# PRBonn/lidar_transfer

Measured on AMD Instinct MI355X. Metric: Mrays/sec, one new ~1M-triangle mesh per scan -> 64x2048 range/label image, higher is better.
Workload: dtype f32; 1 GPU; C2: 64x2048 rays vs 999788-triangle synthetic scene (fov 3.0/-25.0); 1 step = 64 scans, each a new mesh; 48 scenes cycled; parallelism=scan-parallel x1, scans_in_flight=24, scans_per_call=8

## Files before the change

### lidar_transfer_amd/csrc/lt_scatter.hip

```cpp
#include "lt_internal.h"
#include <math.h>
#include <stdlib.h>
#include <string.h>
#include "lt_normalize.h"

#define LT_PI_F 3.14159265358979f
#define LT_BIN_SLACK 4e-3f
#define LT_EMPTY_KEY 0xFFFFFFFFFFFFFFFFull

struct rs_params {
  int nb_az, nb_el;
  float az_scale;
  float az_off;
  float el_lo, el_scale;
  float dev_az, dev_el;
  float dev_fit[2];
  float el_c0, el_c1, az_c0, az_c1;
};

__device__ __forceinline__ float rs_az_off(float phi0, float az_scale) {
  if (!(phi0 == phi0)) return 0.f;
  const float x0 = (phi0 + LT_PI_F) * az_scale;
  return x0 - floorf(x0 + 0.5f);
}

__global__ __launch_bounds__(256) void k_rs_dirs(const float* __restrict__ rays, int n, unsigned flags,
                                                 float4* __restrict__ dirs, float2* __restrict__ ang,
                                                 float* __restrict__ partial) {
  __shared__ float red[4][2];
  float lo = INFINITY, hi = -INFINITY;
  for (int i = blockIdx.x * 256 + threadIdx.x; i < n; i += gridDim.x * 256) {
    const float rx = rays[3 * (size_t)i], ry = rays[3 * (size_t)i + 1], rz = rays[3 * (size_t)i + 2];
    const float D = (rx * rx + ry * ry) + rz * rz;
    const float r0 = lt_rsqrt_seed(D, flags);
    const float r = (1.5f * r0) + (((D * -0.5f) * r0) * (r0 * r0));
    const float dx = rx * r, dy = ry * r, dz = rz * r;
    dirs[i] = make_float4(dx, dy, dz, 0.f);
    const float phi = atan2f(dy, dx), th = atan2f(dz, sqrtf(dx * dx + dy * dy));
    ang[i] = make_float2(phi, th);
    if (th == th) { lo = fminf(lo, th); hi = fmaxf(hi, th); }
  }
#pragma unroll
  for (int o = 32; o > 0; o >>= 1) {
    lo = fminf(lo, __shfl_xor(lo, o, 64));
    hi = fmaxf(hi, __shfl_xor(hi, o, 64));
  }
  if ((threadIdx.x & 63) == 0) { red[threadIdx.x >> 6][0] = lo; red[threadIdx.x >> 6][1] = hi; }
  __syncthreads();
  if (threadIdx.x == 0) {
    partial[2 * blockIdx.x] = fminf(fminf(red[0][0], red[1][0]), fminf(red[2][0], red[3][0]));
    partial[2 * blockIdx.x + 1] = fmaxf(fmaxf(red[0][1], red[1][1]), fmaxf(red[2][1], red[3][1]));
  }
}

__global__ __launch_bounds__(256) void k_rs_fit(const float2* __restrict__ ang, int n, int nb_az0,
                                                rs_params* __restrict__ prm) {
  const float phi0 = n > 0 ? ang[0].x : 0.f;
  float dev[2] = {0.f, 0.f};
  for (int k = 0; k < 2; ++k) {
    const int K = nb_az0 - k;
    if (K < 1) continue;
    const float sc = (float)K / (2.0f * LT_PI_F), off = rs_az_off(phi0, sc);
    for (int i = blockIdx.x * 256 + threadIdx.x; i < n; i += gridDim.x * 256) {
      const float phi = ang[i].x;
      if (phi == phi) {
        const float x = (phi + LT_PI_F) * sc - off;
        dev[k] = fmaxf(dev[k], fabsf(x - floorf(x + 0.5f)));
      }
    }
  }
#pragma unroll
  for (int o = 32; o > 0; o >>= 1) {
    dev[0] = fmaxf(dev[0], __shfl_xor(dev[0], o, 64));
    dev[1] = fmaxf(dev[1], __shfl_xor(dev[1], o, 64));
  }
  if ((threadIdx.x & 63) == 0) {
    atomicMax((int*)&prm->dev_fit[0], __float_as_int(dev[0]));
    atomicMax((int*)&prm->dev_fit[1], __float_as_int(dev[1]));
  }
}

__global__ __launch_bounds__(256) void k_rs_keys(const float2* __restrict__ ang, int n, int nb_az, int nb_el,
                                                 const float* __restrict__ partial, rs_params* __restrict__ prm,
                                                 uint32_t* __restrict__ keys, uint32_t* __restrict__ vals) {
  __shared__ float red[4][2];
  float lo = partial[2 * threadIdx.x], hi = partial[2 * threadIdx.x + 1];
#pragma unroll
  for (int o = 32; o > 0; o >>= 1) {
    lo = fminf(lo, __shfl_xor(lo, o, 64));
    hi = fmaxf(hi, __shfl_xor(hi, o, 64));
  }
  if ((threadIdx.x & 63) == 0) { red[threadIdx.x >> 6][0] = lo; red[threadIdx.x >> 6][1] = hi; }
  __syncthreads();
  lo = fminf(fminf(red[0][0], red[1][0]), fminf(red[2][0], red[3][0]));
  hi = fmaxf(fmaxf(red[0][1], red[1][1]), fmaxf(red[2][1], red[3][1]));
  if (!(lo <= hi)) { lo = 0.f; hi = 0.f; }
  const int nb_max = nb_az;
  if (nb_az >= 5 && prm->dev_fit[1] + 0.01f < prm->dev_fit[0]) nb_az -= 1;
  rs_params p;
  p.nb_az = nb_az; p.nb_el = nb_el;
  p.az_scale = (float)nb_az / (2.0f * LT_PI_F);
  p.az_off = rs_az_off(n > 0 ? ang[0].x : 0.f, p.az_scale);
  p.el_lo = lo;
  p.el_scale = (nb_el > 1 && hi > lo) ? (float)(nb_el - 1) / (hi - lo) : 0.f;
  if (blockIdx.x == 0 && threadIdx.x == 0) {
    prm->nb_az = p.nb_az; prm->nb_el = p.nb_el;
    prm->az_scale = p.az_scale; prm->az_off = p.az_off; prm->el_lo = p.el_lo; prm->el_scale = p.el_scale;
  }
  const int i = blockIdx.x * 256 + threadIdx.x;
  float dev_a = 0.f, dev_e = 0.f;
  if (i < n) {
    const float2 a = ang[i];
    uint32_t key = (uint32_t)nb_max * (uint32_t)nb_el;
    if (a.x == a.x && a.y == a.y) {
      const float x = (a.x + LT_PI_F) * p.az_scale - p.az_off, y = (a.y - p.el_lo) * p.el_scale;
      const float cx = floorf(x + 0.5f);
      const float cy = fminf(fmaxf(floorf(y + 0.5f), 0.f), (float)(nb_el - 1));
      dev_a = fabsf(x - cx);
      dev_e = fabsf(y - cy);
      int ia = (int)cx;
      if (ia < 0) ia += nb_az;
      else if (ia >= nb_az) ia -= nb_az;
      ia = min(max(ia, 0), nb_az - 1);
      key = (uint32_t)cy * (uint32_t)nb_az + (uint32_t)ia;
    }
    keys[i] = key;
    vals[i] = (uint32_t)i;
  }
#pragma unroll
  for (int o = 32; o > 0; o >>= 1) {
    dev_a = fmaxf(dev_a, __shfl_xor(dev_a, o, 64));
    dev_e = fmaxf(dev_e, __shfl_xor(dev_e, o, 64));
  }
  if ((threadIdx.x & 63) == 0) {
    atomicMax((int*)&prm->dev_az, __float_as_int(dev_a));
    atomicMax((int*)&prm->dev_el, __float_as_int(dev_e));
  }
}

__global__ __launch_bounds__(256) void k_rs_starts(const uint32_t* __restrict__ keys, int n, int nbins,
                                                   int* __restrict__ bin_start) {
  const int p = blockIdx.x * 256 + threadIdx.x;
  if (p > n) return;
  const int lo = p == 0 ? 0 : (int)min(keys[p - 1], (uint32_t)nbins) + 1;
  const int hi = p == n ? nbins : (int)min(keys[p], (uint32_t)nbins);
  for (int b = lo; b <= hi; ++b) bin_start[b] = p;
}

struct tri_rec {
  float v0x, v0y, v0z, e1x, e1y, e1z, e2x, e2y, e2z;
};

__device__ __forceinline__ float sc_mt(const tri_rec& T, float ox, float oy, float oz, float dx, float dy, float dz) {
  const float eps = 0.000001f;
  const float hx = dy * T.e2z - dz * T.e2y, hy = dz * T.e2x - dx * T.e2z, hz = dx * T.e2y - dy * T.e2x;
  const float a = (T.e1x * hx + T.e1y * hy) + T.e1z * hz;
  if (a < eps && a > -eps) return NAN;
  const float inv_a = lt_rcp_ieee(a);
  const float sx = ox - T.v0x, sy = oy - T.v0y, sz = oz - T.v0z;
  const float u = ((sx * hx + sy * hy) + sz * hz) * inv_a;
  if (u < 0 || u > 1) return NAN;
  const float qx = sy * T.e1z - sz * T.e1y, qy = sz * T.e1x - sx * T.e1z, qz = sx * T.e1y - sy * T.e1x;
  const float v = ((dx * qx + dy * qy) + dz * qz) * inv_a;
  if (v < 0 || u + v > 1) return NAN;
  const float t = ((T.e2x * qx + T.e2y * qy) + T.e2z * qz) * inv_a;
  if (t < eps) return NAN;
  return t;
}

__device__ __forceinline__ float f_rcp(float x) { return __builtin_amdgcn_rcpf(x); }
__device__ __forceinline__ float f_sqrt(float x) { return __builtin_amdgcn_sqrtf(x); }
__device__ __forceinline__ float f_atan2(float y, float x) {
#pragma clang fp contract(fast)
  const float ax = fabsf(x), ay = fabsf(y);
  const float mx = fmaxf(ax, ay), mn = fminf(ax, ay);
  const float a = mx > 0.f ? mn * f_rcp(mx) : 0.f;
  const float q = a * a;
  float r = a * (0.99997726f + q * (-0.33262347f + q * (0.19354346f + q * (-0.11643287f + q * (0.05265332f + q * -0.01172120f)))));
  r = ay > ax ? 1.57079632679f - r : r;
  r = x < 0.f ? 3.14159265359f - r : r;
  return y < 0.f ? -r : r;
}

__device__ __forceinline__ void f_atan_pair(float za, float ra, float zb, float rb, float& tha, float& thb) {
#pragma clang fp contract(fast)
  const float ta = za * f_rcp(ra), tb = zb * f_rcp(rb);
  const bool easy = fabsf(ta) <= 1.0f && fabsf(tb) <= 1.0f;
  if (__ballot(!easy) == 0ull) {
    const float qa = ta * ta, qb = tb * tb;
    tha = ta * (0.99997726f + qa * (-0.33262347f + qa * (0.19354346f + qa * (-0.11643287f + qa * (0.05265332f + qa * -0.01172120f)))));
    thb = tb * (0.99997726f + qb * (-0.33262347f + qb * (0.19354346f + qb * (-0.11643287f + qb * (0.05265332f + qb * -0.01172120f)))));
  } else {
    tha = f_atan2(za, ra);
    thb = f_atan2(zb, rb);
  }
}

__device__ __forceinline__ float seg_dist2d_sq(float ax, float ay, float bx, float by) {
#pragma clang fp contract(fast)
  const float ex = bx - ax, ey = by - ay;
  const float l2 = ex * ex + ey * ey;
  float t = l2 > 0.f ? -(ax * ex + ay * ey) * f_rcp(l2) : 0.f;
  t = fminf(fmaxf(t, 0.f), 1.f);
  const float cx = ax + t * ex, cy = ay + t * ey;
  return cx * cx + cy * cy;
}

template <class T>
__device__ __forceinline__ unsigned byte_off(unsigned elem) {
  if (sizeof(T) == 12) {
    unsigned r;
    asm("v_lshl_add_u32 %0, %1, 3, %2" : "=v"(r) : "v"(elem), "v"(elem << 2));
    return r;
  }
  return elem * (unsigned)sizeof(T);
}
template <bool WIDE, class T>
__device__ __forceinline__ const T* at(const T* base, unsigned elem) {
  return WIDE ? base + (size_t)elem : (const T*)((const char*)base + byte_off<T>(elem));
}
template <bool WIDE, class T>
__device__ __forceinline__ T* at(T* base, unsigned elem) {
  return WIDE ? base + (size_t)elem : (T*)((char*)base + byte_off<T>(elem));
}
struct f3 { float x, y, z; };
struct i3 { int x, y, z; };

struct bin_rect { int a0, na, e0, e1; };

__device__ __forceinline__ bin_rect tri_bins(const rs_params& P, float x0, float y0, float z0, float x1, float y1,
                                             float z1, float x2, float y2, float z2, float e1x, float e1y, float e2x,
                                             float e2y) {
#pragma clang fp contract(fast)
  bin_rect R;
  R.na = 0;
  const float q0 = x0 * x0 + y0 * y0, q1 = x1 * x1 + y1 * y1, q2 = x2 * x2 + y2 * y2;
  if (!(q0 + q1 + q2 < 1e36f && fabsf(z0) + fabsf(z1) + fabsf(z2) < 1e18f)) {
    const float sum = ((x0 + y0) + (z0 + x1)) + ((y1 + z1) + (x2 + y2)) + z2;
    const float asum = ((fabsf(x0) + fabsf(y0)) + (fabsf(z0) + fabsf(x1))) + ((fabsf(y1) + fabsf(z1)) + (fabsf(x2) + fabsf(y2))) + fabsf(z2);
    if (sum != sum || asum == INFINITY) return R;
    R.e0 = 0; R.e1 = P.nb_el - 1; R.a0 = 0; R.na = P.nb_az;
    return R;
  }
  const float rho_max2 = fmaxf(q0, fmaxf(q1, q2));
  const float rho_max = f_sqrt(rho_max2);
  const float zmin = fminf(z0, fminf(z1, z2)), zmax = fmaxf(z0, fmaxf(z1, z2));
  const float c0 = x0 * y1 - x1 * y0, c1 = x1 * y2 - x2 * y1, c2 = x2 * y0 - x0 * y2;
  const float tol = 1e-6f * rho_max2 + 1e-12f;
  const float cmin = fminf(c0, fminf(c1, c2)), cmax = fmaxf(c0, fmaxf(c1, c2));
  const bool outside = cmin < -tol && cmax > tol;
  bool edge_on = cmin >= -tol && cmax <= tol;
  const float e12x = e2x - e1x, e12y = e2y - e1y;
  const float lmax2 = fmaxf(e1x * e1x + e1y * e1y, fmaxf(e12x * e12x + e12y * e12y, e2x * e2x + e2y * e2y));
  const float qmin = fminf(q0, fminf(q1, q2));
  float rho_edges2;
  if (__ballot(!(lmax2 <= 0.01f * qmin)) == 0ull) {
    rho_edges2 = qmin - 0.25f * lmax2;
  } else {
    rho_edges2 =
        fminf(seg_dist2d_sq(x0, y0, x1, y1), fminf(seg_dist2d_sq(x1, y1, x2, y2), seg_dist2d_sq(x2, y2, x0, y0)));
  }
  const float rho_edges = f_sqrt(rho_edges2);
  const float rho_tiny = 1e-4f * rho_max + 1e-6f;
  if (!outside && rho_edges2 > 4.0f * lmax2) edge_on = true;
  const bool pierced = !(outside || (edge_on && rho_edges > rho_tiny));
  const float rho_min = pierced ? 0.f : rho_edges;
  const float z_near = __builtin_amdgcn_fmed3f(zmin, 0.f, zmax);
  const float dlo2 = fmaxf((pierced ? 0.f : rho_edges2) + z_near * z_near, 0.0025f);
  const float pad = 3e-4f + 2e-4f * __builtin_amdgcn_rsqf(dlo2);
  const float pad_az = 3e-4f + 2e-4f * __builtin_amdgcn_rsqf(fmaxf(rho_edges2, 0.0025f));
  float th_hi, th_lo;
  f_atan_pair(zmax, zmax > 0.f ? rho_min : rho_max, zmin, zmin < 0.f ? rho_min : rho_max, th_hi, th_lo);
  th_hi += pad;
  th_lo -= pad;
  const float fe0 = ceilf(th_lo * P.el_scale + P.el_c0), fe1 = floorf(th_hi * P.el_scale + P.el_c1);
  if (!(fe1 >= 0.f) || !(fe0 <= (float)(P.nb_el - 1)) || !(fe0 <= fe1)) return R;
  R.e0 = (int)fmaxf(fe0, 0.f);
  R.e1 = (int)fminf(fe1, (float)(P.nb_el - 1));
  if (pierced || rho_min <= rho_tiny || P.nb_az < 4) {
    R.a0 = 0;
    R.na = P.nb_az;
    return R;
  }
  float a_lo, a_hi;
  if (!edge_on) {
    const bool l0 = c0 >= 0.f && c2 <= 0.f, l1 = c1 >= 0.f && c0 <= 0.f;
    const bool h0 = c0 <= 0.f && c2 >= 0.f, h1 = c1 <= 0.f && c0 >= 0.f;
    a_lo = f_atan2(l0 ? y0 : (l1 ? y1 : y2), l0 ? x0 : (l1 ? x1 : x2));
    a_hi = f_atan2(h0 ? y0 : (h1 ? y1 : y2), h0 ? x0 : (h1 ? x1 : x2));
    if (a_hi < a_lo) a_hi += 2.0f * LT_PI_F;
  } else {
    const float p0 = f_atan2(y0, x0), p1 = f_atan2(y1, x1), p2 = f_atan2(y2, x2);
    const float lo = fminf(p0, fminf(p1, p2)), hi = fmaxf(p0, fmaxf(p1, p2));
    const float mid = (p0 + p1 + p2) - lo - hi;
    const float g0 = mid - lo, g1 = hi - mid, g2 = 2.0f * LT_PI_F - (hi - lo);
    if (g2 >= g0 && g2 >= g1) { a_lo = lo; a_hi = hi; }
    else if (g0 >= g1) { a_lo = mid; a_hi = lo + 2.0f * LT_PI_F; }
    else { a_lo = hi; a_hi = mid + 2.0f * LT_PI_F; }
  }
  a_lo -= pad_az;
  a_hi += pad_az;
  const float fa0 = ceilf(a_lo * P.az_scale + P.az_c0);
  const float fa1 = floorf(a_hi * P.az_scale + P.az_c1);
  const int na = (int)(fa1 - fa0) + 1;
  if (!(na >= 1)) return R;
  if (na >= P.nb_az) { R.a0 = 0; R.na = P.nb_az; return R; }
  int a0 = (int)fa0;
  if (a0 < 0) a0 += P.nb_az;
  else if (a0 >= P.nb_az) a0 -= P.nb_az;
  R.a0 = a0;
  R.na = na;
  return R;
}

#define LT_GRID_EMPTY (-1)
#define LT_GRID_MULTI (-2)
template <bool WIDE>
__device__ __forceinline__ void sc_hit(float t, int ray, int face, unsigned long long* __restrict__ cell) {
  if (t < 999999999.f) atomicMin(at<WIDE>(cell, (unsigned)ray), ((unsigned long long)__float_as_uint(t) << 32) | (unsigned)face);
}
template <bool WIDE>
__device__ __forceinline__ void sc_test_cell(const tri_rec& T, int face, const float4 g,
                                             const float4* __restrict__ sdirs, float ox, float oy, float oz,
                                             unsigned long long* __restrict__ cell, unsigned& n_tests) {
  const int w = __float_as_int(g.w);
  if (w != LT_GRID_MULTI) {
    n_tests += w >= 0 ? 1u : 0u;
    sc_hit<WIDE>(sc_mt(T, ox, oy, oz, g.x, g.y, g.z), w, face, cell);
  } else {
    for (int k = __float_as_int(g.x), e = __float_as_int(g.y); k < e; ++k) {
      const float4 d = *at<WIDE>(sdirs, (unsigned)k);
      ++n_tests;
      sc_hit<WIDE>(sc_mt(T, ox, oy, oz, d.x, d.y, d.z), __float_as_int(d.w), face, cell);
    }
  }
}

__global__ __launch_bounds__(256) void k_rs_sortdirs(const float4* __restrict__ dirs,
                                                     const uint32_t* __restrict__ bin_rays, int n,
                                                     float4* __restrict__ sdirs) {
  const int k = blockIdx.x * 256 + threadIdx.x;
  if (k >= n) return;
  const int ray = (int)bin_rays[k];
  float4 d = dirs[ray];
  d.w = __int_as_float(ray);
  sdirs[k] = d;
}

__global__ __launch_bounds__(256) void k_rs_grid(const int* __restrict__ bin_start,
                                                 const float4* __restrict__ sdirs, int nbins,
                                                 float4* __restrict__ grid) {
  const int b = blockIdx.x * 256 + threadIdx.x;
  if (b >= nbins) return;
  const int s = bin_start[b], e = bin_start[b + 1];
  float4 g = make_float4(0.f, 0.f, 0.f, __int_as_float(LT_GRID_EMPTY));
  if (e - s == 1) g = sdirs[s];
  else if (e - s > 1) g = make_float4(__int_as_float(s), __int_as_float(e), 0.f, __int_as_float(LT_GRID_MULTI));
  grid[b] = g;
}

#define LT_SC_BIG 512
#define LT_SC_CAP_SINGLE 1536
#define LT_SC_CAP_BATCH 8192
#ifndef LT_SC_SLICE
#define LT_SC_SLICE 512
#endif

#ifndef LT_SC_T
#define LT_SC_T 448
#endif
#define LT_SC_T2 (LT_SC_T - 256)
static_assert(LT_SC_T >= 256 && LT_SC_T <= 512 && LT_SC_T2 % 64 == 0, "LT_SC_T: 256, 320, 384, 448 or 512");

struct sc_shared {
  float4 q0[LT_SC_T], q1[LT_SC_T];
  float2 q2[LT_SC_T];
  unsigned pre[513];
  unsigned wsum[4];
  int kept;
};

struct sc_one { int cnt; unsigned a0; };

template <bool PUSH>
__device__ __forceinline__ sc_one sc_record_into(float4* s_q0, float4* s_q1, float2* s_q2, int slot, int f, const f3 A,
                                                 const f3 Bv, const f3 C, float ox, float oy, float oz, const rs_params& P,
                                                 int* __restrict__ large, int* __restrict__ large_count) {
  sc_one r;
  r.cnt = 0; r.a0 = 0;
  const float v0x = A.x, v0y = A.y, v0z = A.z, v1x = Bv.x, v1y = Bv.y, v1z = Bv.z;
  const float v2x = C.x, v2y = C.y, v2z = C.z;
  const float e1x = v1x - v0x, e1y = v1y - v0y, e2x = v2x - v0x, e2y = v2y - v0y;
  const bin_rect R = tri_bins(P, v0x - ox, v0y - oy, v0z - oz, v1x - ox, v1y - oy, v1z - oz, v2x - ox, v2y - oy,
                              v2z - oz, e1x, e1y, e2x, e2y);
  if (R.na > 0) {
    const int c32 = R.na * (R.e1 - R.e0 + 1);
    if (c32 > LT_SC_BIG) {
      if (PUSH) large[atomicAdd(large_count, 1)] = f;
    } else {
      r.cnt = c32;
      r.a0 = (unsigned)R.a0;
      s_q0[slot] = make_float4(v0x, v0y, v0z, e1x);
      s_q1[slot] = make_float4(e1y, v1z - v0z, e2x, e2y);
      s_q2[slot] = make_float2(v2z - v0z, __int_as_float((R.na - 1) | (R.e0 << 9)));
    }
  }
  return r;
}
template <bool PUSH>
__device__ __forceinline__ sc_one sc_record(sc_shared& S, int slot, int f, const f3 A, const f3 Bv, const f3 C, float ox,
                                            float oy, float oz, const rs_params& P, int* __restrict__ large,
                                            int* __restrict__ large_count) {
  return sc_record_into<PUSH>(S.q0, S.q1, S.q2, slot, f, A, Bv, C, ox, oy, oz, P, large, large_count);
}

template <bool PUSH, bool WIDE>
__device__ __forceinline__ void sc_setup(sc_shared& S, const float* __restrict__ verts, const int* __restrict__ faces,
                                         int n_verts, int n_faces, int first, float ox, float oy, float oz,
                                         const rs_params& P, int* __restrict__ large, int* __restrict__ large_count,
                                         unsigned* __restrict__ flags, sc_one& rA, sc_one& rB) {
  const int tid = threadIdx.x;
  rA.cnt = 0; rA.a0 = 0; rB.cnt = 0; rB.a0 = 0;
  const int fA = first + tid, fB = first + 256 + tid;
  const bool hasA = fA < n_faces, hasB = LT_SC_T2 > 0 && tid < LT_SC_T2 && fB < n_faces;
  if (n_verts <= 0) {
    if (PUSH && (hasA || hasB)) atomicOr(flags, LT_FLAG_BAD_INDEX);
    return;
  }
  const i3 iA = *at<WIDE>((const i3*)faces, (unsigned)(hasA ? fA : 0));
  i3 iB = iA;
  if (LT_SC_T2 > 0) iB = *at<WIDE>((const i3*)faces, (unsigned)(hasB ? fB : 0));
  const unsigned nv = (unsigned)n_verts;
  const bool okA = hasA && (unsigned)iA.x < nv && (unsigned)iA.y < nv && (unsigned)iA.z < nv;
  const bool okB = hasB && (unsigned)iB.x < nv && (unsigned)iB.y < nv && (unsigned)iB.z < nv;
  const f3 A0 = *at<WIDE>((const f3*)verts, okA ? (unsigned)iA.x : 0u);
  const f3 A1 = *at<WIDE>((const f3*)verts, okA ? (unsigned)iA.y : 0u);
  const f3 A2 = *at<WIDE>((const f3*)verts, okA ? (unsigned)iA.z : 0u);
  f3 B0 = A0, B1 = A1, B2 = A2;
  if (LT_SC_T2 > 0) {
    B0 = *at<WIDE>((const f3*)verts, okB ? (unsigned)iB.x : 0u);
    B1 = *at<WIDE>((const f3*)verts, okB ? (unsigned)iB.y : 0u);
    B2 = *at<WIDE>((const f3*)verts, okB ? (unsigned)iB.z : 0u);
  }
  if (PUSH && ((hasA && !okA) || (hasB && !okB))) atomicOr(flags, LT_FLAG_BAD_INDEX);
  if (okA) rA = sc_record<PUSH>(S, tid, fA, A0, A1, A2, ox, oy, oz, P, large, large_count);
  if (LT_SC_T2 > 0 && okB) rB = sc_record<PUSH>(S, 256 + tid, fB, B0, B1, B2, ox, oy, oz, P, large, large_count);
}

__device__ __forceinline__ void sc_prefix(sc_shared& S, const sc_one rA, const sc_one rB, int& preA, int& preB, int& total) {
  const int tid = threadIdx.x, lane = tid & 63, wave = tid >> 6;
  unsigned inc = (unsigned)rA.cnt | ((unsigned)rB.cnt << 16);
  asm volatile(
      "s_nop 1\n\tv_add_u32_dpp %0, %0, %0 row_shr:1 row_mask:0xf bank_mask:0xf bound_ctrl:0\n\t"
      "s_nop 1\n\tv_add_u32_dpp %0, %0, %0 row_shr:2 row_mask:0xf bank_mask:0xf bound_ctrl:0\n\t"
      "s_nop 1\n\tv_add_u32_dpp %0, %0, %0 row_shr:4 row_mask:0xf bank_mask:0xf bound_ctrl:0\n\t"
      "s_nop 1\n\tv_add_u32_dpp %0, %0, %0 row_shr:8 row_mask:0xf bank_mask:0xf bound_ctrl:0\n\t"
      "s_nop 1\n\tv_add_u32_dpp %0, %0, %0 row_bcast:15 row_mask:0xa bank_mask:0xf\n\t"
      "s_nop 1\n\tv_add_u32_dpp %0, %0, %0 row_bcast:31 row_mask:0xc bank_mask:0xf\n\t"
      "s_nop 1"
      : "+v"(inc));
  if (lane == 63) S.wsum[wave] = inc;
  __syncthreads();
  int woffA = 0, woffB = 0, totA = 0, totB = 0;
#pragma unroll
  for (int w = 0; w < 4; ++w) {
    const unsigned ws = S.wsum[w];
    const int a = (int)(ws & 0xFFFFu), b = (int)(ws >> 16);
    if (w < wave) { woffA += a; woffB += b; }
    totA += a; totB += b;
  }
  total = totA + totB;
  preA = woffA + (int)(inc & 0xFFFFu) - rA.cnt;
  preB = totA + woffB + (int)(inc >> 16) - rB.cnt;
  S.pre[tid] = ((unsigned)preA << 13) | rA.a0;
  if (LT_SC_T2 > 0 && tid < LT_SC_T2) S.pre[256 + tid] = ((unsigned)preB << 13) | rB.a0;
  else S.pre[256 + tid] = (256 + tid == LT_SC_T) ? ((unsigned)total << 13) : 0xFFFFFFFFu;
  if (tid == 255) S.pre[512] = LT_SC_T == 512 ? ((unsigned)total << 13) : 0xFFFFFFFFu;
}

template <bool COUNT, bool WIDE, int NT, int NE>
__device__ __forceinline__ void sc_round_robin(const unsigned* s_pre, const float4* s_q0, const float4* s_q1,
                                               const float2* s_q2, const rs_params& P, const float4* __restrict__ grid,
                                               const float4* __restrict__ sdirs, unsigned long long* __restrict__ cell,
                                               int first_face, int c_begin, int c_end, int tix, float ox, float oy, float oz,
                                               unsigned& n_tests, unsigned& n_cand) {
  auto ldu = [](const unsigned* arr, unsigned j4) { return *(const unsigned*)((const char*)arr + j4); };
  auto ldq = [](const float4* arr, unsigned j4) { return *(const float4*)((const char*)arr + 4u * j4); };
  auto ld2 = [](const float2* arr, unsigned j4) { return *(const float2*)((const char*)arr + 2u * j4); };
  const unsigned pre0 = s_pre[0];
  auto locate = [&](int c, unsigned& j4, float2& q2) -> int {
    const unsigned ck = ((unsigned)c << 13) | 0x1FFFu;
    j4 = 0;
    unsigned base = pre0;
#pragma unroll
    for (unsigned step4 = 2u * NE; step4 >= 4; step4 >>= 1) {
      const unsigned v = ldu(s_pre, j4 + step4);
      const bool take = v <= ck;
      j4 = take ? j4 + step4 : j4;
      base = take ? v : base;
    }
    const int local = c - (int)(base >> 13);
    q2 = ld2(s_q2, j4);
    const int pk = __float_as_int(q2.y);
    const int na = (pk & 511) + 1;
    const int row = (int)(((float)local + 0.5f) * f_rcp((float)na));
    int az = (int)(base & 0x1FFFu) + (local - __mul24(row, na));
    if (az >= P.nb_az) az -= P.nb_az;
    return __mul24((pk >> 9) + row, P.nb_az) + az;
  };
  int c = c_begin + tix;
  if (c < c_end) {
    unsigned j4;
    float2 q2;
    float4 g = *at<false>(grid, (unsigned)locate(c, j4, q2));
    for (;;) {
      const int cn = c + NT;
      unsigned jn4 = 0;
      float2 q2n = make_float2(0.f, 0.f);
      float4 gn = make_float4(0.f, 0.f, 0.f, 0.f);
      if (__ballot(cn < c_end) != 0ull) gn = *at<false>(grid, (unsigned)locate(min(cn, c_end - 1), jn4, q2n));
      const float4 q0 = ldq(s_q0, j4), q1 = ldq(s_q1, j4);
      tri_rec T;
      T.v0x = q0.x; T.v0y = q0.y; T.v0z = q0.z;
      T.e1x = q0.w; T.e1y = q1.x; T.e1z = q1.y;
      T.e2x = q1.z; T.e2y = q1.w; T.e2z = q2.x;
      if (COUNT) ++n_cand;
      sc_test_cell<WIDE>(T, first_face + (int)(j4 >> 2), g, sdirs, ox, oy, oz, cell, n_tests);
      if (cn >= c_end) break;
      c = cn; j4 = jn4; g = gn; q2 = q2n;
    }
  }
}

template <bool COUNT>
__device__ __forceinline__ void sc_count(unsigned n_tests, unsigned n_cand, unsigned long long* __restrict__ counters) {
  if (COUNT) {
    unsigned long long vt = n_tests, vc = n_cand;
#pragma unroll
    for (int o = 32; o > 0; o >>= 1) { vt += __shfl_xor(vt, o, 64); vc += __shfl_xor(vc, o, 64); }
    if ((threadIdx.x & 63) == 0) { atomicAdd(&counters[1], vt); atomicAdd(&counters[0], vc); }
  }
}

#ifndef LT_SC_MAX_BATCH
#define LT_SC_MAX_BATCH 8
#endif
struct sc_job {
  const float* verts; const int* faces; const int* colors; const float* rem;
  rs_params P; const float4* grid; const float4* sdirs; const float4* dirs;
  unsigned long long* cell; int* large; int* large_count; int2* slices;
  unsigned* flags; unsigned long long* counters;
  float* endpoints; int* endcolors; float* range; float* endrem; int* tri;
  float ox, oy, oz;
  int n_verts, n_faces, n_rays, cap_slices;
  unsigned out_flags;
};
struct sc_batch {
  int n;
  int tris_blocks, resolve_blocks;
  int cap;
  int rest_blocks;
  int tris_block0[LT_SC_MAX_BATCH];
  int resolve_block0[LT_SC_MAX_BATCH];
  sc_job job[LT_SC_MAX_BATCH];
};
__device__ __forceinline__ int sc_find_job(const int (&block0)[LT_SC_MAX_BATCH], int block) {
  int j = 0;
#pragma unroll
  for (int k = 1; k < LT_SC_MAX_BATCH; ++k) j += block >= block0[k] ? 1 : 0;
  return j;
}


template <bool COUNT, bool WIDE>
__global__ __launch_bounds__(256) void k_sc_tris(const sc_batch B) {
  __shared__ sc_shared S;
  const int j = sc_find_job(B.tris_block0, (int)blockIdx.x);
  const sc_job& J = B.job[j];
  const int lb = (int)blockIdx.x - B.tris_block0[j];
  const int tid = threadIdx.x;
  const int first = lb * LT_SC_T;
  const rs_params P = J.P;
  const float ox = J.ox, oy = J.oy, oz = J.oz;
  sc_one rA, rB;
  sc_setup<true, WIDE>(S, J.verts, J.faces, J.n_verts, J.n_faces, first, ox, oy, oz, P, J.large, J.large_count, J.flags, rA,
                       rB);
  int total, preA, preB;
  sc_prefix(S, rA, rB, preA, preB, total);
  if (total < B.cap) {
    if (tid == 255) S.kept = total;
  } else {
    const bool crossA = preA < B.cap && preA + rA.cnt >= B.cap;
    const bool crossB = LT_SC_T2 > 0 && tid < LT_SC_T2 && preB < B.cap && preB + rB.cnt >= B.cap;
    if (crossA || crossB) {
      int kept = crossA ? preA + rA.cnt : preB + rB.cnt;
      const int n_sl = (total - kept + LT_SC_SLICE - 1) / LT_SC_SLICE;
      if (n_sl > 0) {
        const int base = atomicAdd(&J.large_count[1], n_sl);
        if (base + n_sl <= J.cap_slices) {
          for (int k = 0; k < n_sl; ++k) J.slices[base + k] = make_int2(lb, kept + k * LT_SC_SLICE);
        } else {
          atomicSub(&J.large_count[1], n_sl);
          kept = total;
        }
      }
      S.kept = kept;
    }
  }
  __syncthreads();
  const int kept = S.kept;
  unsigned n_tests = 0, n_cand = 0;
  sc_round_robin<COUNT, WIDE, 256, (LT_SC_T > 256 ? 512 : 256)>(S.pre, S.q0, S.q1, S.q2, P, J.grid, J.sdirs, J.cell, first, 0,
                                                                kept, tid, ox, oy, oz, n_tests, n_cand);
  sc_count<COUNT>(n_tests, n_cand, J.counters);
}

#define LT_SC_REST_BLOCKS 512
#define LT_SC_REST_BLOCKS_BATCH 128
#define LT_SC_PARTS 8
template <bool COUNT, bool WIDE>
__global__ __launch_bounds__(256) void k_sc_rest(const sc_batch B) {
  __shared__ sc_shared S;
  const int rest_blocks = B.rest_blocks;
  const sc_job& J = B.job[blockIdx.x / rest_blocks];
  const int rb = blockIdx.x % rest_blocks;
  if (J.n_faces <= 0) return;
  const float* __restrict__ verts = J.verts;
  const int* __restrict__ faces = J.faces;
  const float4* __restrict__ grid = J.grid;
  const float4* __restrict__ sdirs = J.sdirs;
  unsigned long long* __restrict__ cell = J.cell;
  const float ox = J.ox, oy = J.oy, oz = J.oz;
  const rs_params P = J.P;
  const int n_large = J.large_count[0], n_slices = min(J.large_count[1], J.cap_slices);
  if (COUNT && rb == 0 && threadIdx.x == 0) J.counters[3] = (unsigned long long)n_large | ((unsigned long long)n_slices << 32);
  unsigned n_tests = 0, n_cand = 0;
  for (int q = rb; q < n_slices; q += rest_blocks) {
    const int2 sl = J.slices[q];
    const int first = sl.x * LT_SC_T;
    sc_one rA, rB;
    sc_setup<false, WIDE>(S, verts, faces, J.n_verts, J.n_faces, first, ox, oy, oz, P, nullptr, nullptr, nullptr, rA, rB);
    int total, preA, preB;
    sc_prefix(S, rA, rB, preA, preB, total);
    __syncthreads();
    sc_round_robin<COUNT, WIDE, 256, (LT_SC_T > 256 ? 512 : 256)>(S.pre, S.q0, S.q1, S.q2, P, grid, sdirs, cell, first, sl.y,
                                                                  min(sl.y + LT_SC_SLICE, total), (int)threadIdx.x, ox, oy,
                                                                  oz, n_tests, n_cand);
    __syncthreads();
  }
  const int lane = threadIdx.x & 63;
  const int wave0 = rb * 4 + (threadIdx.x >> 6), nwaves = rest_blocks * 4;
  for (int v = wave0; v < n_large * LT_SC_PARTS; v += nwaves) {
    const int q = v / LT_SC_PARTS, part = v - q * LT_SC_PARTS;
    const int f = J.large[q];
    const float* pa = verts + 3 * (size_t)faces[3 * (size_t)f];
    const float* pb = verts + 3 * (size_t)faces[3 * (size_t)f + 1];
    const float* pc = verts + 3 * (size_t)faces[3 * (size_t)f + 2];
    tri_rec T;
    T.v0x = pa[0]; T.v0y = pa[1]; T.v0z = pa[2];
    const float v1x = pb[0], v1y = pb[1], v1z = pb[2], v2x = pc[0], v2y = pc[1], v2z = pc[2];
    T.e1x = v1x - T.v0x; T.e1y = v1y - T.v0y; T.e1z = v1z - T.v0z;
    T.e2x = v2x - T.v0x; T.e2y = v2y - T.v0y; T.e2z = v2z - T.v0z;
    const bin_rect R = tri_bins(P, T.v0x - ox, T.v0y - oy, T.v0z - oz, v1x - ox, v1y - oy, v1z - oz, v2x - ox,
                                v2y - oy, v2z - oz, T.e1x, T.e1y, T.e2x, T.e2y);
    const int total = R.na > 0 ? R.na * (R.e1 - R.e0 + 1) : 0;
    const int parts = min(max((total + 1023) / 1024, 1), LT_SC_PARTS);
    if (part >= parts) continue;
    for (int w = part * 64 + lane; w < total; w += 64 * parts) {
      const int row = w / R.na;
      const int e = R.e0 + row;
      int az = R.a0 + (w - row * R.na);
      if (az >= P.nb_az) az -= P.nb_az;
      if (COUNT) ++n_cand;
      sc_test_cell<WIDE>(T, f, grid[e * P.nb_az + az], sdirs, ox, oy, oz, cell, n_tests);
    }
  }
  sc_count<COUNT>(n_tests, n_cand, J.counters);
}

template <bool COUNT>
__global__ __launch_bounds__(256) void k_sc_resolve(const sc_batch B) {
  const int j = sc_find_job(B.resolve_block0, (int)blockIdx.x);
  const sc_job& J = B.job[j];
  const int ray = ((int)blockIdx.x - B.resolve_block0[j]) * 256 + threadIdx.x;
  unsigned long long* __restrict__ cell = J.cell;
  const int* __restrict__ faces = J.faces;
  float* __restrict__ endpoints = J.endpoints;
  int* __restrict__ endcolors = J.endcolors;
  float* __restrict__ range = J.range;
  float* __restrict__ endrem = J.endrem;
  int* __restrict__ tri_out = J.tri;
  const unsigned flags = J.out_flags;
  if (ray == 0) { J.large_count[0] = 0; J.large_count[1] = 0; }
  bool hit = false;
  if (ray < J.n_rays) {
    const unsigned long long key = cell[ray];
    const float4 d = J.dirs[ray];
    cell[ray] = LT_EMPTY_KEY;
    hit = key != LT_EMPTY_KEY;
    if (hit) {
      const float t = __uint_as_float((unsigned)(key >> 32));
      const int face = (int)(unsigned)(key & 0xFFFFFFFFull);
      const int i0 = faces[3 * (size_t)face], i1 = faces[3 * (size_t)face + 1], i2 = faces[3 * (size_t)face + 2];
      const int* __restrict__ colors = J.colors;
      const float* __restrict__ rem = J.rem;
      const bool label = (flags & LT_TRACE_LABEL_IMAGE) != 0;
      int c0 = 0, c1 = 0, c2 = 0;
      float r0 = 0.f, r1 = 0.f, r2 = 0.f;
      if (endcolors) {
        c2 = colors[3 * (size_t)i0 + 2];
        if (!label) { c0 = colors[3 * (size_t)i0]; c1 = colors[3 * (size_t)i0 + 1]; }
      }
      if (endrem) { r0 = rem[i0]; r1 = rem[i1]; r2 = rem[i2]; }
      if (endpoints) {
        endpoints[3 * (size_t)ray] = J.ox + d.x * t;
        endpoints[3 * (size_t)ray + 1] = J.oy + d.y * t;
        endpoints[3 * (size_t)ray + 2] = J.oz + d.z * t;
      }
      if (endcolors) {
        if (label) {
          endcolors[ray] = (int)(float)c2;
        } else {
          endcolors[3 * (size_t)ray] = (int)(float)c0;
          endcolors[3 * (size_t)ray + 1] = (int)(float)c1;
          endcolors[3 * (size_t)ray + 2] = (int)(float)c2;
        }
      }
      if (endrem) endrem[ray] = ((r0 + r1) + r2) / 3.0f;
      if (range) range[ray] = t;
      if (tri_out) tri_out[ray] = face;
    } else if (flags & LT_TRACE_WRITE_MISSES) {
      if (endpoints) { endpoints[3 * (size_t)ray] = 0.f; endpoints[3 * (size_t)ray + 1] = 0.f; endpoints[3 * (size_t)ray + 2] = 0.f; }
      if (endcolors) {
        if (flags & LT_TRACE_LABEL_IMAGE) endcolors[ray] = 0;
        else { endcolors[3 * (size_t)ray] = 0; endcolors[3 * (size_t)ray + 1] = 0; endcolors[3 * (size_t)ray + 2] = 0; }
      }
      if (endrem) endrem[ray] = 0.f;
      if (range) range[ray] = 0.f;
      if (tri_out) tri_out[ray] = -1;
    }
  }
  if (COUNT) {
    unsigned long long vh = hit ? 1u : 0u;
#pragma unroll
    for (int o = 32; o > 0; o >>= 1) vh += __shfl_xor(vh, o, 64);
    if ((threadIdx.x & 63) == 0) atomicAdd(&J.counters[2], vh);
  }
}

void lt_sort_pairs(uint32_t* keys[2], uint32_t* vals[2], uint32_t* hist, int n, int key_bits, hipStream_t stream,
                   int* out_buffer);

static void rs_derive(rs_params& p) {
  const float de = p.dev_el + LT_BIN_SLACK, da = p.dev_az + LT_BIN_SLACK;
  p.el_c0 = -p.el_lo * p.el_scale - de;
  p.el_c1 = -p.el_lo * p.el_scale + de;
  p.az_c0 = LT_PI_F * p.az_scale - p.az_off - da;
  p.az_c1 = LT_PI_F * p.az_scale - p.az_off + da;
}

struct lt_rayset {
  int device;
  int n_rays, height, nb_az, nb_el;
  unsigned norm_flags;
  float4* dirs;
  float2* ang;
  float* partial;
  rs_params* prm;
  rs_params prm_host;
  uint32_t* keys[2];
  uint32_t* vals[2];
  uint32_t* hist;
  int* bin_start;
  uint32_t* bin_rays;
  float4* sdirs;
  float4* grid;
};

static void rs_free(lt_rayset* r) {
  void* ps[] = {r->grid, r->sdirs, r->dirs, r->ang, r->partial, r->prm, r->keys[0], r->keys[1], r->vals[0], r->vals[1], r->hist,
                r->bin_start};
  for (void* p : ps)
    if (p) (void)hipFree(p);
}

extern "C" int lt_rayset_destroy(lt_rayset* r) {
  if (!r) return LT_OK;
  (void)hipSetDevice(r->device);
  (void)hipDeviceSynchronize();
  rs_free(r);
  free(r);
  return LT_OK;
}

extern "C" int lt_rayset_create_dev(lt_rayset** out, const float* rays, int n_rays, int height, unsigned flags,
                                    void* stream_) {
  if (!out || n_rays < 0 || height <= 0 || (n_rays > 0 && !rays)) {
    lt_set_error("lt_rayset_create_dev: invalid argument (n_rays=%d height=%d)", n_rays, height);
    return LT_ERR_INVALID_ARG;
  }
  *out = nullptr;
  hipStream_t stream = (hipStream_t)stream_;
  int device = 0;
  LT_HIP(hipGetDevice(&device));
  lt_rayset* r = (lt_rayset*)calloc(1, sizeof(lt_rayset));
  if (!r) return LT_ERR_NO_MEMORY;
  r->device = device;
  const int W = n_rays / height;
  const int n = W * height;
  r->n_rays = n;
  r->height = height;
  r->norm_flags = flags & (LT_TRACE_NORM_EXACT | LT_TRACE_NORM_AMD);
  r->nb_az = W < 1 ? 1 : (W > 8192 ? 8192 : W);
  r->nb_el = height > 4096 ? 4096 : height;
  const size_t nbins = (size_t)r->nb_az * r->nb_el + 1;
  const size_t nn = n > 0 ? n : 1;
  const int nb = (int)((nn + LT_SORT_TILE - 1) / LT_SORT_TILE);
  int rc = LT_OK;
#define RS_ALLOC(ptr, bytes)                                                  \
  if (rc == LT_OK && hipMalloc((void**)&(ptr), (bytes)) != hipSuccess) {      \
    lt_set_error("lt_rayset_create_dev: hipMalloc of %zu bytes failed", (size_t)(bytes)); \
    rc = LT_ERR_NO_MEMORY;                                                    \
  }
  RS_ALLOC(r->dirs, nn * sizeof(float4));
  RS_ALLOC(r->ang, nn * sizeof(float2));
  RS_ALLOC(r->sdirs, nn * sizeof(float4));
  RS_ALLOC(r->partial, 2 * 256 * sizeof(float));
  RS_ALLOC(r->prm, sizeof(rs_params));
  for (int k = 0; k < 2; ++k) {
    RS_ALLOC(r->keys[k], nn * sizeof(uint32_t));
    RS_ALLOC(r->vals[k], nn * sizeof(uint32_t));
  }
  RS_ALLOC(r->hist, ((size_t)1024 * nb + 1024) * sizeof(uint32_t));
  RS_ALLOC(r->bin_start, (nbins + 1) * sizeof(int));
  RS_ALLOC(r->grid, nbins * sizeof(float4));
#undef RS_ALLOC
  if (rc != LT_OK) {
    rs_free(r);
    free(r);
    return rc;
  }
  if (hipMemsetAsync(r->prm, 0, sizeof(rs_params), stream) != hipSuccess) {
    lt_set_error("lt_rayset_create_dev: hipMemsetAsync failed");
    rs_free(r);
    free(r);
    return LT_ERR_HIP;
  }
  hipLaunchKernelGGL(k_rs_dirs, dim3(256), dim3(256), 0, stream, rays, n, r->norm_flags, r->dirs, r->ang, r->partial);
  hipLaunchKernelGGL(k_rs_fit, dim3(64), dim3(256), 0, stream, r->ang, n, r->nb_az, r->prm);
  hipLaunchKernelGGL(k_rs_keys, dim3((n + 255) / 256 > 0 ? (n + 255) / 256 : 1), dim3(256), 0, stream, r->ang, n,
                     r->nb_az, r->nb_el, r->partial, r->prm, r->keys[0], r->vals[0]);
  int buf = 0;
  if (n > 0) lt_sort_pairs(r->keys, r->vals, r->hist, n, 30, stream, &buf);
  r->bin_rays = r->vals[buf];
  hipLaunchKernelGGL(k_rs_starts, dim3((n + 1 + 255) / 256), dim3(256), 0, stream, r->keys[buf], n, (int)nbins,
                     r->bin_start);
  if (n > 0)
    hipLaunchKernelGGL(k_rs_sortdirs, dim3((n + 255) / 256), dim3(256), 0, stream, r->dirs, r->bin_rays, n, r->sdirs);
  hipLaunchKernelGGL(k_rs_grid, dim3((unsigned)((nbins + 255) / 256)), dim3(256), 0, stream, r->bin_start, r->sdirs,
                     (int)nbins, r->grid);
  const hipError_t le = hipGetLastError();
  if (le != hipSuccess) {
    lt_set_error("lt_rayset_create_dev: kernel launch failed: %s", hipGetErrorString(le));
    (void)hipStreamSynchronize(stream);
    rs_free(r);
    free(r);
    return LT_ERR_HIP;
  }
  if (hipStreamSynchronize(stream) != hipSuccess ||
      hipMemcpy(&r->prm_host, r->prm, sizeof(rs_params), hipMemcpyDeviceToHost) != hipSuccess) {
    lt_set_error("lt_rayset_create_dev: ray set preparation failed: %s", hipGetErrorString(hipGetLastError()));
    rs_free(r);
    free(r);
    return LT_ERR_HIP;
  }
  rs_derive(r->prm_host);
  *out = r;
  return LT_OK;
}

static int sc_reserve(lt_scene* s, int n_faces, int n_rays, hipStream_t stream) {
  if (!s->sc_large_count) {
    LT_HIP(hipMalloc((void**)&s->sc_large_count, 4 * sizeof(int)));
    LT_HIP(hipMemsetAsync(s->sc_large_count, 0, 4 * sizeof(int), stream));
  }
  if (n_rays > s->sc_cap_cells) {
    if (s->sc_cell) {
      LT_HIP(hipDeviceSynchronize());
      (void)hipFree(s->sc_cell);
      s->sc_cell = nullptr;
      s->sc_cap_cells = 0;
    }
    LT_HIP(hipMalloc((void**)&s->sc_cell, (size_t)n_rays * sizeof(unsigned long long)));
    s->sc_cap_cells = n_rays;
    LT_HIP(hipMemsetAsync(s->sc_cell, 0xFF, (size_t)n_rays * sizeof(unsigned long long), stream));
  }
  if (n_faces > s->sc_cap_queue) {
    if (s->sc_large || s->sc_slices) {
      LT_HIP(hipDeviceSynchronize());
      (void)hipFree(s->sc_large);
      (void)hipFree(s->sc_slices);
      s->sc_large = nullptr;
      s->sc_slices = nullptr;
      s->sc_cap_queue = 0;
    }
    const size_t cap = (size_t)n_faces + n_faces / 4 + 1024;
    LT_HIP(hipMalloc((void**)&s->sc_large, cap * sizeof(int)));
    LT_HIP(hipMalloc((void**)&s->sc_slices, cap * sizeof(int2)));
    s->sc_cap_queue = (int)cap;
  }
  return LT_OK;
}

struct sc_item {
  lt_scene* s;
  lt_rayset* r;
  const float* origin;
  float* endpoints; int* endcolors; float* range; float* endrem; int* tri;
};

static int sc_launch_batch(const sc_item* it, int n_items, unsigned flags, hipStream_t stream, bool count,
                           lt_scene* probe) {
  sc_batch B;
  memset(&B, 0, sizeof(B));
  for (int k = 0; k < LT_SC_MAX_BATCH; ++k) B.tris_block0[k] = B.resolve_block0[k] = 0x7fffffff;
  static const bool force_wide = getenv("LIDARHIP_FORCE_WIDE") != nullptr;
  bool wide = force_wide;
  int tb = 0, rb = 0;
  for (int i = 0; i < n_items; ++i) {
    lt_scene* s = it[i].s;
    lt_rayset* r = it[i].r;
    const int n = s->n_faces, R = r->n_rays;
    if (R <= 0) continue;
    LT_CHECK(sc_reserve(s, n, R, stream));
    sc_job& J = B.job[B.n++];
    J.verts = s->verts; J.faces = s->faces; J.colors = s->colors; J.rem = s->rem;
    J.P = r->prm_host; J.grid = r->grid; J.sdirs = r->sdirs; J.dirs = r->dirs;
    J.cell = s->sc_cell; J.large = s->sc_large; J.large_count = s->sc_large_count; J.slices = s->sc_slices;
    J.flags = s->flags; J.counters = s->counters;
    J.endpoints = it[i].endpoints; J.endcolors = it[i].endcolors; J.range = it[i].range; J.endrem = it[i].endrem;
    J.tri = it[i].tri;
    J.ox = it[i].origin[0]; J.oy = it[i].origin[1]; J.oz = it[i].origin[2];
    J.n_verts = s->n_verts; J.n_faces = n; J.n_rays = R; J.cap_slices = s->sc_cap_queue;
    J.out_flags = flags;
    B.tris_block0[B.n - 1] = tb;
    B.resolve_block0[B.n - 1] = rb;
    tb += (n + LT_SC_T - 1) / LT_SC_T;
    rb += (R + 255) / 256;
    wide = wide || (size_t)n * 12 >= (1ull << 32) || (size_t)s->n_verts * 12 >= (1ull << 32) ||
           (size_t)R * 16 >= (1ull << 32);
  }
  if (B.n == 0) return LT_OK;
  B.tris_blocks = tb;
  B.resolve_blocks = rb;
  static const int env_cap = []() {
    const char* e = getenv("LIDARHIP_SC_CAP");
    return e ? atoi(e) : 0;
  }();
  B.cap = env_cap > 0 ? env_cap : (n_items > 1 ? LT_SC_CAP_BATCH : LT_SC_CAP_SINGLE);
  static const int env_rest = []() {
    const char* e = getenv("LIDARHIP_SC_REST_BLOCKS");
    return e ? atoi(e) : 0;
  }();
  B.rest_blocks = env_rest > 0 ? env_rest : (n_items > 1 ? LT_SC_REST_BLOCKS_BATCH : LT_SC_REST_BLOCKS);
  const dim3 b(256);
#define SC_LAUNCH(KERNEL, GRID) \
  do { \
    if (count && wide) hipLaunchKernelGGL((KERNEL<true, true>), GRID, b, 0, stream, B); \
    else if (count) hipLaunchKernelGGL((KERNEL<true, false>), GRID, b, 0, stream, B); \
    else if (wide) hipLaunchKernelGGL((KERNEL<false, true>), GRID, b, 0, stream, B); \
    else hipLaunchKernelGGL((KERNEL<false, false>), GRID, b, 0, stream, B); \
  } while (0)
  if (tb > 0) {
    if (probe && probe->probe[0]) LT_HIP(hipEventRecord(probe->probe[0], stream));
    SC_LAUNCH(k_sc_tris, dim3(tb));
    if (probe) {
      if (probe->probe[1]) LT_HIP(hipEventRecord(probe->probe[1], stream));
      probe->probe[0] = probe->probe[1] = nullptr;
    }
    SC_LAUNCH(k_sc_rest, dim3(B.n * B.rest_blocks));
  }
#undef SC_LAUNCH
  if (count) hipLaunchKernelGGL(k_sc_resolve<true>, dim3(rb), b, 0, stream, B);
  else hipLaunchKernelGGL(k_sc_resolve<false>, dim3(rb), b, 0, stream, B);
  LT_HIP(hipGetLastError());
  return LT_OK;
}

extern "C" int lt_scene_render_dev(lt_scene* s, lt_rayset* r, const float* origin, float* endpoints, int* endcolors,
                                   float* range, float* endrem, int* tri, unsigned flags, void* stream_,
                                   lt_stats* stats) {
  if (!s || !r || !origin) {
    lt_set_error("lt_scene_render_dev: NULL scene / rayset / origin");
    return LT_ERR_INVALID_ARG;
  }
  if (s->device != r->device) {
    lt_set_error("lt_scene_render_dev: scene on device %d, rayset on device %d", s->device, r->device);
    return LT_ERR_INVALID_ARG;
  }
  hipStream_t stream = (hipStream_t)stream_;
  LT_HIP(hipSetDevice(s->device));
  s->last_stream = stream;
  const int n = s->n_faces, R = r->n_rays;
  const bool timed = stats != nullptr, count = (flags & LT_TRACE_COUNT) != 0;
  s->stats.n_rays = R;
  s->stats.n_faces = n;
  if (R > 0) {
    if (count) LT_HIP(hipMemsetAsync(s->counters, 0, 4 * sizeof(unsigned long long), stream));
    if (timed) LT_HIP(hipEventRecord(s->ev[7], stream));
    const sc_item it = {s, r, origin, endpoints, endcolors, range, endrem, tri};
    LT_CHECK(sc_launch_batch(&it, 1, flags, stream, count, count ? nullptr : s));
    if (timed) LT_HIP(hipEventRecord(s->ev[8], stream));
  }
  if (timed || count) {
    LT_HIP(hipStreamSynchronize(stream));
    if (timed && R > 0) LT_HIP(hipEventElapsedTime(&s->stats.ms_trace, s->ev[7], s->ev[8]));
    if (count && R > 0) {
      unsigned long long c[4];
      LT_HIP(hipMemcpy(c, s->counters, sizeof(c), hipMemcpyDeviceToHost));
      s->stats.nodes_visited = c[0];
      s->stats.tris_tested = c[1];
      s->stats.n_hits = (int)c[2];
      s->stats.stack_overflows = 0;
      s->stats.entries_culled = 0;
    }
    if (stats) *stats = s->stats;
  }
  return LT_OK;
}

extern "C" int lt_scene_render_batch_dev(int n_scans, lt_scene* const* scenes, lt_rayset* const* raysets,
                                         const float* origins, float* const* endpoints, int* const* endcolors,
                                         float* const* range, float* const* endrem, int* const* tri, unsigned flags,
                                         void* stream_) {
  if (n_scans < 0 || n_scans > LT_SC_MAX_BATCH || (n_scans > 0 && (!scenes || !raysets || !origins))) {
    lt_set_error("lt_scene_render_batch_dev: invalid argument (n_scans=%d, at most %d per call)", n_scans,
                 LT_SC_MAX_BATCH);
    return LT_ERR_INVALID_ARG;
  }
  if (flags & LT_TRACE_COUNT) {
    lt_set_error("lt_scene_render_batch_dev: LT_TRACE_COUNT is a single-scan diagnostic (lt_scene_render_dev)");
    return LT_ERR_INVALID_ARG;
  }
  if (n_scans == 0) return LT_OK;
  hipStream_t stream = (hipStream_t)stream_;
  sc_item it[LT_SC_MAX_BATCH];
  lt_scene* probe = nullptr;
  for (int i = 0; i < n_scans; ++i) {
    if (!scenes[i] || !raysets[i] || scenes[i]->device != raysets[i]->device ||
        scenes[i]->device != scenes[0]->device) {
      lt_set_error("lt_scene_render_batch_dev: scan %d: NULL scene / rayset, or not all on one device", i);
      return LT_ERR_INVALID_ARG;
    }
    for (int k = 0; k < i; ++k)
      if (scenes[k] == scenes[i]) {
        lt_set_error("lt_scene_render_batch_dev: scans %d and %d are the same scene (a scene renders one scan at a time)", k, i);
        return LT_ERR_INVALID_ARG;
      }
    it[i] = {scenes[i], raysets[i], origins + 3 * i, endpoints ? endpoints[i] : nullptr,
             endcolors ? endcolors[i] : nullptr, range ? range[i] : nullptr, endrem ? endrem[i] : nullptr,
             tri ? tri[i] : nullptr};
    scenes[i]->last_stream = stream;
    scenes[i]->stats.n_rays = raysets[i]->n_rays;
    scenes[i]->stats.n_faces = scenes[i]->n_faces;
    if (!probe && scenes[i]->probe[0]) probe = scenes[i];
  }
  LT_HIP(hipSetDevice(scenes[0]->device));
  return sc_launch_batch(it, n_scans, flags, stream, false, probe ? probe : scenes[0]);
}

extern "C" int lt_debug_scatter_queues(lt_scene* s, int* out2) {
  if (!s || !out2) return LT_ERR_INVALID_ARG;
  LT_HIP(hipSetDevice(s->device));
  LT_HIP(hipDeviceSynchronize());
  unsigned long long c = 0;
  LT_HIP(hipMemcpy(&c, s->counters + 3, sizeof(c), hipMemcpyDeviceToHost));
  out2[0] = (int)(c & 0xFFFFFFFFull);
  out2[1] = (int)(c >> 32);
  return LT_OK;
}
extern "C" int lt_debug_scatter_large(lt_scene* s, int* out, int n) {
  if (!s || !out || n < 0 || n > s->sc_cap_queue) return LT_ERR_INVALID_ARG;
  LT_HIP(hipSetDevice(s->device));
  LT_HIP(hipDeviceSynchronize());
  LT_HIP(hipMemcpy(out, s->sc_large, (size_t)n * sizeof(int), hipMemcpyDeviceToHost));
  return LT_OK;
}
```

Baseline: 11800 Mrays/s.

## Tighten elevation bin padding and use polynomial atan for small triangles

```diff
diff --git a/lidar_transfer_amd/csrc/lt_scatter.hip b/lidar_transfer_amd/csrc/lt_scatter.hip
--- a/lidar_transfer_amd/csrc/lt_scatter.hip
+++ b/lidar_transfer_amd/csrc/lt_scatter.hip
@@ -6,6 +6,10 @@
 
 #define LT_PI_F 3.14159265358979f
 #define LT_BIN_SLACK 4e-3f
+#define LT_PAD_ANG 4e-5f
+#define LT_PAD_MT 6e-5f
+#define LT_PAD_ILL 3e-4f
+#define LT_OMEGA2_MAX 0.0081f
 #define LT_EMPTY_KEY 0xFFFFFFFFFFFFFFFFull
 
 struct rs_params {
@@ -242,6 +246,8 @@
     R.e0 = 0; R.e1 = P.nb_el - 1; R.a0 = 0; R.na = P.nb_az;
     return R;
   }
+  const float t0 = z0 * __builtin_amdgcn_rsqf(q0), t1 = z1 * __builtin_amdgcn_rsqf(q1), t2 = z2 * __builtin_amdgcn_rsqf(q2);
+  const float ta = fmaxf(t0, fmaxf(t1, t2)), tb = fminf(t0, fminf(t1, t2));
   const float rho_max2 = fmaxf(q0, fmaxf(q1, q2));
   const float rho_max = f_sqrt(rho_max2);
   const float zmin = fminf(z0, fminf(z1, z2)), zmax = fmaxf(z0, fmaxf(z1, z2));
@@ -266,11 +272,26 @@
   const bool pierced = !(outside || (edge_on && rho_edges > rho_tiny));
   const float rho_min = pierced ? 0.f : rho_edges;
   const float z_near = __builtin_amdgcn_fmed3f(zmin, 0.f, zmax);
-  const float dlo2 = fmaxf((pierced ? 0.f : rho_edges2) + z_near * z_near, 0.0025f);
-  const float pad = 3e-4f + 2e-4f * __builtin_amdgcn_rsqf(dlo2);
-  const float pad_az = 3e-4f + 2e-4f * __builtin_amdgcn_rsqf(fmaxf(rho_edges2, 0.0025f));
+  const float dm2 = (pierced ? 0.f : rho_edges2) + z_near * z_near;
+  const float inv_d = __builtin_amdgcn_rsqf(fmaxf(dm2, 0.0025f));
+  const float det = z0 * c1 + (z1 * c2 + z2 * c0);
+  const float dz = zmax - zmin, L2 = lmax2 + dz * dz;
+  const float zabs = fmaxf(zmax, -zmin);
+  const bool well = (rho_max2 + zabs * zabs) * L2 * (21.f * 5.9604645e-8f) <= LT_PAD_MT * ((dm2 * inv_d) * fabsf(det));
+  const float pad_c = well ? LT_PAD_ANG + LT_PAD_MT : LT_PAD_ILL;
+  float pad = pad_c + 2e-4f * inv_d;
+  const float pad_az = pad_c + 2e-4f * __builtin_amdgcn_rsqf(fmaxf(rho_edges2, 0.0025f));
   float th_hi, th_lo;
-  f_atan_pair(zmax, zmax > 0.f ? rho_min : rho_max, zmin, zmin < 0.f ? rho_min : rho_max, th_hi, th_lo);
+  const bool small_tri = !pierced && rho_edges > rho_tiny && L2 <= LT_OMEGA2_MAX * dm2 && zabs * zabs <= rho_edges2 &&
+                         dm2 >= 0.0025f;
+  if (__ballot(!small_tri) == 0ull) {
+    const float qa = ta * ta, qb = tb * tb;
+    th_hi = ta * (0.99997726f + qa * (-0.33262347f + qa * (0.19354346f + qa * (-0.11643287f + qa * (0.05265332f + qa * -0.01172120f)))));
+    th_lo = tb * (0.99997726f + qb * (-0.33262347f + qb * (0.19354346f + qb * (-0.11643287f + qb * (0.05265332f + qb * -0.01172120f)))));
+    pad += (0.13f * fmaxf(ta, -tb) + 0.001f) * ((L2 * inv_d) * inv_d);
+  } else {
+    f_atan_pair(zmax, zmax > 0.f ? rho_min : rho_max, zmin, zmin < 0.f ? rho_min : rho_max, th_hi, th_lo);
+  }
   th_hi += pad;
   th_lo -= pad;
   const float fe0 = ceilf(th_lo * P.el_scale + P.el_c0), fe1 = floorf(th_hi * P.el_scale + P.el_c1);
@@ -619,7 +640,7 @@
 #define LT_SC_REST_BLOCKS_BATCH 128
 #define LT_SC_PARTS 8
 template <bool COUNT, bool WIDE>
-__global__ __launch_bounds__(256) void k_sc_rest(const sc_batch B) {
+__global__ __launch_bounds__(256) __attribute__((amdgpu_waves_per_eu(8, 8))) void k_sc_rest(const sc_batch B) {
   __shared__ sc_shared S;
   const int rest_blocks = B.rest_blocks;
   const sc_job& J = B.job[blockIdx.x / rest_blocks];
@@ -648,7 +669,7 @@
                                                                   oz, n_tests, n_cand);
     __syncthreads();
   }
-  const int lane = threadIdx.x & 63;
+  const int lane = (int)__lane_id();
   const int wave0 = rb * 4 + (threadIdx.x >> 6), nwaves = rest_blocks * 4;
   for (int v = wave0; v < n_large * LT_SC_PARTS; v += nwaves) {
     const int q = v / LT_SC_PARTS, part = v - q * LT_SC_PARTS;
```

Measured after the change: 11700 Mrays/s. No clear change (-0.9%).
